# baekingeol/Probing-RAG

Measured on NVIDIA B200. Metric: bm25_top10_queries_per_sec, higher is better.
Workload: dtype f32

## Files before the change

include/probing_rag.h:

```cpp
#ifndef PROBING_RAG_H
#define PROBING_RAG_H

#include <stddef.h>
#include <stdint.h>

#ifdef __cplusplus
extern "C" {
#endif

#define PR_VERSION 201

#define PR_OK 0
#define PR_EINVAL (-1)
#define PR_ECUDA (-2)
#define PR_ERANGE (-3)
#define PR_EWORKSPACE (-4)
#define PR_EUNSUPPORTED (-5)

#define PR_MAX_K 128

typedef struct pr_index pr_index_t;
typedef void *pr_stream_t;

typedef struct pr_bm25_tuning {
// ... 38 lines not shown

int32_t pr_bm25_num_launches(const pr_index_t *index, int32_t n_queries, int32_t k, int64_t n_docs);
size_t pr_bm25_theta_offset(const pr_index_t *index, int32_t n_queries, int32_t k);
int pr_bm25_topk_range(pr_index_t *index, int32_t n_queries, const int64_t *q_indptr_dev,
                       const int32_t *q_terms_dev, int64_t n_q_terms, int32_t k, float *out_scores_dev,
                       int32_t *out_doc_ids_dev, void *workspace_dev, size_t workspace_bytes,
                       int32_t launch_begin, int32_t launch_end, pr_stream_t stream);

size_t pr_bm25_running_scores_offset(const pr_index_t *index, int32_t n_queries, int32_t k);
int pr_bm25_raise_union_bound(pr_index_t *index, int32_t n_queries, int32_t k, const float *gathered_scores_dev,
                              int32_t n_lists, void *workspace_dev, size_t workspace_bytes, pr_stream_t stream);

#define PR_MAX_PEERS 15
typedef struct pr_ipc_handle { unsigned char bytes[64]; } pr_ipc_handle_t;
int pr_peer_alloc(int device, size_t bytes, void **out_dev, pr_ipc_handle_t *out_handle);
int pr_peer_open(int device, const pr_ipc_handle_t *handle, void **out_dev);
int pr_peer_close(void *dev);
int pr_peer_free(void *dev);
int pr_index_set_peer_thetas(pr_index_t *index, float *local_dev, int64_t capacity, int32_t n_peers,
                             float *const *peer_bases_host, void *peer_table_dev);

int pr_bm25_status(const void *workspace_dev, pr_stream_t stream);

int pr_index_set_profiling(pr_index_t *index, int enable);
int pr_bm25_profile(pr_index_t *index, float *score_ms, int32_t *score_launches);

int64_t pr_bm25_last_launches(const pr_index_t *index);

int pr_topk_merge(int32_t n_queries, int32_t k, int32_t n_lists, const float *scores_dev,
                  const int32_t *ids_dev, float *out_scores_dev, int32_t *out_ids_dev,
                  pr_stream_t stream);

#define PR_PROBER_MAX 8

typedef struct pr_prober_set {
    int32_t n_probers;
    int32_t d_model;
    int32_t hidden;
    const float *w1_rowsum;
    const float *b1;
    const float *ln1_w, *ln1_b;
    const float *b2;
    const float *ln2_w, *ln2_b;
    const float *w3, *b3;
    const void *w1_hi, *w1_lo;
    const void *w2_hi, *w2_lo;
// ... 59 lines not shown
```

probing_rag_b200/_lib.py:

```python
from __future__ import annotations

import ctypes
import os

PKG_DIR = os.path.dirname(os.path.abspath(__file__))
LIB_PATH = os.environ.get("PR_LIB_PATH") or os.path.join(PKG_DIR, "libprobingrag.so")

PR_OK, PR_EINVAL, PR_ECUDA, PR_ERANGE, PR_EWORKSPACE, PR_EUNSUPPORTED = 0, -1, -2, -3, -4, -5
PR_MAX_K = 128
PR_PROBER_MAX = 8
PR_MAX_PEERS = 15
PR_FLAT_MAX_LISTS = 32
PR_METRIC_INNER_PRODUCT, PR_METRIC_L2 = 0, 1

c_i32, c_i64, c_f32, c_vp, c_sz = ctypes.c_int32, ctypes.c_int64, ctypes.c_float, ctypes.c_void_p, ctypes.c_size_t


class Tuning(ctypes.Structure):
    _fields_ = [("subs_per_item", c_i32), ("warps_per_cta", c_i32), ("docs_per_launch", c_i32),
                ("min_items", c_i32), ("items_per_warp", c_i32), ("tile_epochs", c_i32),
                ("batch_variant", c_i32)]


class AuxInfo(ctypes.Structure):
    _fields_ = [("table_rows", c_i32), ("hot_rows", c_i32), ("n_sub_tiles", c_i32),
                ("table_min_df", c_i64), ("hot_min_df", c_i64), ("hot_stream_bytes", c_i64),
                ("cold_stream_bytes", c_i64)]


class ProberSet(ctypes.Structure):
    _fields_ = [("n_probers", c_i32), ("d_model", c_i32), ("hidden", c_i32),
                ("w1_rowsum", c_vp), ("b1", c_vp),
                ("ln1_w", c_vp), ("ln1_b", c_vp), ("b2", c_vp),
                ("ln2_w", c_vp), ("ln2_b", c_vp), ("w3", c_vp), ("b3", c_vp),
                ("w1_hi", c_vp), ("w1_lo", c_vp), ("w2_hi", c_vp), ("w2_lo", c_vp)]


class FlatTuning(ctypes.Structure):
    _fields_ = [("first_chunk_rows", c_i64), ("growth", c_i32), ("cand_capacity", c_i32)]


class FlatStats(ctypes.Structure):
    _fields_ = [("launches", c_i64), ("chunks", c_i64), ("candidates", c_i64), ("max_candidates", c_i64),
                ("fallback_queries", c_i64)]


SIGNATURES = {
    "pr_version": (ctypes.c_int, []),
    "pr_last_error": (ctypes.c_char_p, []),
    "pr_index_create": (ctypes.c_int, [ctypes.POINTER(c_vp), ctypes.c_int, c_i64, c_i32, c_i32, c_i32, c_i64,
                                       c_vp, c_vp, c_vp]),
    "pr_index_destroy": (ctypes.c_int, [c_vp]),
    "pr_index_aux_bytes": (c_sz, [c_vp, c_sz]),
    "pr_index_build_aux": (ctypes.c_int, [c_vp, c_vp, c_sz, c_vp]),
    "pr_index_aux_info": (ctypes.c_int, [c_vp, ctypes.POINTER(AuxInfo)]),
    "pr_index_set_tuning": (ctypes.c_int, [c_vp, ctypes.POINTER(Tuning)]),
    "pr_index_get_tuning": (ctypes.c_int, [c_vp, ctypes.POINTER(Tuning)]),
    "pr_bm25_workspace_bytes": (c_sz, [c_vp, c_i32, c_i32]),
    "pr_bm25_topk": (ctypes.c_int, [c_vp, c_i32, c_vp, c_vp, c_i64, c_i32, c_vp, c_vp, c_vp, c_sz, c_vp]),
    "pr_bm25_num_launches": (c_i32, [c_vp, c_i32, c_i32, c_i64]),
    "pr_bm25_theta_offset": (c_sz, [c_vp, c_i32, c_i32]),
    "pr_bm25_running_scores_offset": (c_sz, [c_vp, c_i32, c_i32]),
    "pr_bm25_raise_union_bound": (ctypes.c_int, [c_vp, c_i32, c_i32, c_vp, c_i32, c_vp, c_sz, c_vp]),
    "pr_bm25_topk_range": (ctypes.c_int, [c_vp, c_i32, c_vp, c_vp, c_i64, c_i32, c_vp, c_vp, c_vp, c_sz, c_i32, c_i32,
                                          c_vp]),
    "pr_peer_alloc": (ctypes.c_int, [ctypes.c_int, c_sz, ctypes.POINTER(c_vp), ctypes.c_char_p]),
    "pr_peer_open": (ctypes.c_int, [ctypes.c_int, ctypes.c_char_p, ctypes.POINTER(c_vp)]),
    "pr_peer_close": (ctypes.c_int, [c_vp]),
    "pr_peer_free": (ctypes.c_int, [c_vp]),
    "pr_index_set_peer_thetas": (ctypes.c_int, [c_vp, c_vp, c_i64, c_i32, ctypes.POINTER(c_vp), c_vp]),
    "pr_bm25_status": (ctypes.c_int, [c_vp, c_vp]),
    "pr_bm25_last_launches": (c_i64, [c_vp]),
    "pr_index_set_profiling": (ctypes.c_int, [c_vp, ctypes.c_int]),
    "pr_bm25_profile": (ctypes.c_int, [c_vp, ctypes.POINTER(c_f32), ctypes.POINTER(c_i32)]),
    "pr_topk_merge": (ctypes.c_int, [c_i32, c_i32, c_i32, c_vp, c_vp, c_vp, c_vp, c_vp]),
    "pr_prober_workspace_bytes": (c_sz, [c_i32, c_i32, c_i32, c_i32]),
    "pr_pool_accumulate": (ctypes.c_int, [c_vp, c_i32, c_i32, c_i32, c_i32, c_vp, c_i32, c_i32, c_i32, c_i64, c_i64,
                                          c_vp, c_vp]),
    "pr_prober_forward": (ctypes.c_int, [ctypes.POINTER(ProberSet), c_i32, c_vp, c_i32, ctypes.c_double, c_i32, c_vp, c_vp,
                                         c_vp, c_vp, c_vp, c_vp, c_sz, c_vp]),
    "pr_flat_create": (ctypes.c_int, [ctypes.POINTER(c_vp), ctypes.c_int, c_vp, c_i64, c_i32]),
    "pr_flat_create_metric": (ctypes.c_int, [ctypes.POINTER(c_vp), ctypes.c_int, c_vp, c_i64, c_i32, ctypes.c_int]),
    "pr_flat_destroy": (ctypes.c_int, [c_vp]),
    "pr_flat_aux_bytes": (c_sz, [c_vp]),
    "pr_flat_build_aux": (ctypes.c_int, [c_vp, c_vp, c_sz, c_vp]),
    "pr_flat_set_tuning": (ctypes.c_int, [c_vp, ctypes.POINTER(FlatTuning)]),
    "pr_flat_get_tuning": (ctypes.c_int, [c_vp, ctypes.POINTER(FlatTuning)]),
    "pr_flat_workspace_bytes": (c_sz, [c_vp, c_i32, c_i32]),
    "pr_flat_search": (ctypes.c_int, [c_vp, c_i32, c_vp, c_i32, c_vp, c_vp, c_vp, c_sz, c_vp]),
    "pr_flat_last_stats": (ctypes.c_int, [c_vp, c_vp, c_i32, c_i32, ctypes.POINTER(FlatStats), c_vp]),
    "pr_flat_merge": (ctypes.c_int, [c_i32, c_i32, c_i32, c_vp, c_vp, ctypes.POINTER(c_i64), c_vp, c_vp, c_vp]),
    "pr_flat_merge_metric": (ctypes.c_int, [c_i32, c_i32, c_i32, c_vp, c_vp, ctypes.POINTER(c_i64), c_vp, c_vp, c_vp,
                                            ctypes.c_int]),
}
# ... 31 lines not shown
```

probing_rag_b200/csrc/bm25.cu:

```cuda
#include <string.h>

#include <vector>

#include "common.cuh"
#include "bm25_lean.cuh"
#include "bm25_kernels.h"

namespace {

__device__ __forceinline__ void fill_zero_tail(float *out_s, int32_t *out_d, int K, int nvalid, int doc_id_base, int n_docs)
{
    int cand = 0;
    for (int pos = nvalid; pos < K; ++pos) {
        while (cand < n_docs) {
            bool listed = false;
            for (int i = 0; i < nvalid; ++i)
                if (out_d[i] == cand + doc_id_base) listed = true;
            if (!listed) break;
            ++cand;
        }
        if (cand >= n_docs) break;
        out_s[pos] = 0.f;
        out_d[pos] = cand + doc_id_base;
        ++cand;
// ... 254 lines not shown
        const float *ps = gs + ((size_t)g * B + q) * K;
        bool done = false;
#pragma unroll
        for (int e = 0; e < E; ++e) {
            const int i0 = e * 32;
            if (done || i0 >= K) break;
            const float es = i0 + lane < K ? ps[i0 + lane] : -1.f;
            const int n = min(32, K - i0);
            for (int i = 0; i < n; ++i) {
                const float bs = __shfl_sync(PR_FULL_MASK, es, i);
                const int bd = g * K + i0 + i;
                if (bs < 0.f || !pr_beats(bs, bd, ks, kd)) {
                    done = true;
                    break;
                }
                L.insert(bs, bd, lane);
                L.kth(K, ks, kd);
            }
        }
    }
    if (ks > 0.f) prw::raise_theta(theta, nullptr, 0, q, ks, lane);
}

__global__ void bm25_init_kernel(float *run_s, int32_t *run_d, float *theta, int64_t n_run, int B, int32_t *counters,
                                 int n_counters, int32_t *status)
{
    const int64_t i = (int64_t)blockIdx.x * blockDim.x + threadIdx.x;
    if (i < n_run) {
        run_s[i] = PR_SENT_SCORE;
        run_d[i] = PR_SENT_DOC;
    }
    if (i < B && theta) theta[i] = PR_SENT_SCORE;
    if (i < n_counters) counters[i] = 0;
    if (i == 0) *status = 0;
}

__global__ void bm25_fill_kernel(float *p, int64_t n, float v)
{
    for (int64_t i = (int64_t)blockIdx.x * blockDim.x + threadIdx.x; i < n; i += (int64_t)gridDim.x * blockDim.x) p[i] = v;
}

__global__ void bm25_validate_kernel(const int64_t *indptr, const int32_t *doc_ids,
                                     const float *weights, int n_terms, int64_t nnz, int n_docs,
                                     int32_t *bad)
{
    const int64_t stride = (int64_t)gridDim.x * blockDim.x;
    const int64_t i0 = (int64_t)blockIdx.x * blockDim.x + threadIdx.x;
    for (int64_t t = i0; t < n_terms; t += stride) {
        const int64_t b = indptr[t], e = indptr[t + 1];
        if (b > e || b < 0 || e > nnz) atomicOr(bad, 1);
    }
    if (i0 == 0 && (indptr[0] != 0 || indptr[n_terms] != nnz)) atomicOr(bad, 1);
    uint32_t wmin = 0xffffffffu, wmax = 0u;
    for (int64_t p = i0; p < nnz; p += stride) {
        const int32_t d = doc_ids[p];
        const float w = weights[p];
        if (d < 0 || d >= n_docs) atomicOr(bad, 2);
// ... 23 lines not shown
}

}

constexpr int kNwChoices = 3;
constexpr int kEChoices = 3;

struct pr_index {
    int device;
    int64_t n_docs_global;
    int32_t doc_id_base, n_docs, n_terms;
    int64_t nnz;
    const int64_t *indptr;
    const int32_t *doc_ids;
    const float *weights;
    pr_bm25_tuning_t tuning;
    int num_sms;
    int64_t last_launches;
    int profiling;
    std::vector<cudaEvent_t> ev;
    int ev_used;
    const int32_t *heavy_row;
    const uint32_t *tp;
    int32_t n_rows, n_sub;
    int64_t heavy_min_df;
    const int32_t *hot_of_row;
    const uint32_t *hot_off;
    int32_t n_hot;
    int64_t hot_min_df, hot_stream_bytes;
    const unsigned char *cold_stream;
    uint32_t hot_base_g;
    int occ[kNwChoices][kEChoices][3];
    float max_weight;
    bool scale_ok;
    float *peer_local;
    float *const *peer_table;
    int32_t n_peers;
    int64_t peer_capacity;
    uint64_t peer_calls;
    int union_lists;
};

namespace {

struct Layout {
    int n_chunks, C, L;
// ... 157 lines not shown
    }
    pr_index *ix = new pr_index();
    memset(ix->occ, 0, sizeof(ix->occ));
    ix->peer_local = nullptr;
    ix->peer_table = nullptr;
    ix->n_peers = 0;
    ix->peer_capacity = 0;
    ix->peer_calls = 0;
    ix->union_lists = 1;
    ix->device = device;
    ix->n_docs_global = n_docs_global;
    ix->doc_id_base = doc_id_base;
    ix->n_docs = n_docs;
    ix->n_terms = n_terms;
    ix->nnz = nnz;
    ix->indptr = indptr_dev;
    ix->doc_ids = doc_ids_dev;
    ix->weights = weights_dev;
    ix->last_launches = 0;
    ix->profiling = 0;
    ix->ev_used = 0;
    ix->heavy_row = nullptr;
    ix->tp = nullptr;
    ix->n_rows = 0;
    ix->n_sub = (int32_t)(((int64_t)n_docs + prw::kSub - 1) >> prw::kSubShift);
    ix->heavy_min_df = 0;
    ix->hot_of_row = nullptr;
    ix->hot_off = nullptr;
    ix->n_hot = 0;
    ix->hot_min_df = 0;
    ix->hot_stream_bytes = 0;
    ix->cold_stream = nullptr;
    ix->hot_base_g = 0;
    {
        float wmin = 0.f, wmax = 0.f;
        if (nnz > 0) {
            memcpy(&wmin, &h_bad3[1], 4);
            memcpy(&wmax, &h_bad3[2], 4);
        }
        ix->max_weight = wmax;
        ix->scale_ok = nnz > 0 && wmin >= 9.313225746154785e-10f && wmax <= 256.f;
    }
    default_tuning(&ix->tuning);
    cudaDeviceProp prop;
    PR_CUDA_CHECK(cudaGetDeviceProperties(&prop, device));
    ix->num_sms = prop.multiProcessorCount;
    *out = ix;
    return PR_OK;
}

extern "C" int pr_index_destroy(pr_index_t *index)
{
    if (index)
        for (cudaEvent_t e : index->ev) cudaEventDestroy(e);
    delete index;
    return PR_OK;
}

extern "C" size_t pr_index_aux_bytes(const pr_index_t *index, size_t table_budget_bytes)
{
    if (!index) return 0;
    const size_t fixed = align_up((size_t)index->n_terms * 4, 256) + align_up(((size_t)index->n_terms / 1024 + 2) * 4, 256) + 256;
    return fixed + align_up((size_t)index->nnz * 8 + 256, 256) + align_up(table_budget_bytes, 256);
}

extern "C" int pr_index_build_aux(pr_index_t *index, void *aux_dev, size_t aux_bytes, pr_stream_t stream)
{
    if (!index || !aux_dev) {
        pr_set_error("pr_index_build_aux: null argument");
        return PR_EINVAL;
    }
    cudaStream_t st = (cudaStream_t)stream;
    const int nt = index->n_terms;
    const int n_blocks = (nt + 1023) / 1024;
    unsigned char *p = (unsigned char *)aux_dev;
    size_t o = 0;
    int32_t *heavy_row = (int32_t *)(p + o);  o = align_up(o + (size_t)nt * 4, 256);
    int32_t *block_cnt = (int32_t *)(p + o);  o = align_up(o + ((size_t)nt / 1024 + 2) * 4, 256);
    int32_t *count = (int32_t *)(p + o);      o += 256;
    unsigned char *cold = p + o;              o += align_up((size_t)index->nnz * 8 + 256, 256);
    if (o > aux_bytes) {
        pr_set_error("pr_index_build_aux: aux buffer of %zu bytes, need at least %zu (tables + 8 bytes per posting)", aux_bytes, o);
        return PR_EWORKSPACE;
    }
    const size_t budget = aux_bytes - o;
    size_t table_bytes = budget / 5;
    if (table_bytes < ((size_t)16 << 20)) table_bytes = budget < ((size_t)16 << 20) ? budget : ((size_t)16 << 20);
    const size_t per_row = ((size_t)index->n_sub + 1) * 4 + 4;
    int64_t min_df = prw::kLightDf;
    int32_t rows = 0;
    for (;;) {
        PR_CUDA_CHECK(cudaMemsetAsync(count, 0, 4, st));
        if (nt > 0) prw::count_heavy_kernel<<<296, 256, 0, st>>>(index->indptr, nt, min_df, count);
        PR_CUDA_CHECK(cudaGetLastError());
        PR_CUDA_CHECK(cudaMemcpyAsync(&rows, count, 4, cudaMemcpyDeviceToHost, st));
        PR_CUDA_CHECK(cudaStreamSynchronize(st));
        if ((size_t)rows * per_row + 1024 <= table_bytes || rows == 0) break;
        min_df *= 2;
    }
    int32_t *row_term = (int32_t *)(p + o);   o = align_up(o + (size_t)(rows > 0 ? rows : 1) * 4, 256);
    uint32_t *tp = (uint32_t *)(p + o);       o = align_up(o + (size_t)rows * ((size_t)index->n_sub + 1) * 4, 256);
    if (nt > 0) {
        prw::heavy_block_count_kernel<<<n_blocks, 1024, 0, st>>>(index->indptr, nt, min_df, block_cnt);
        prw::heavy_block_scan_kernel<<<1, 32, 0, st>>>(block_cnt, n_blocks);
        prw::heavy_assign_kernel<<<n_blocks, 1024, 0, st>>>(index->indptr, nt, min_df, block_cnt, heavy_row, row_term);
        if (rows > 0)
            prw::tp_fill_kernel<<<2368, 256, 0, st>>>(index->indptr, index->doc_ids, row_term, rows, index->n_sub, tp);
    }
    if (index->nnz > 0)
        prl::cold_fill_kernel<<<2368, 256, 0, st>>>(index->doc_ids, index->weights, index->nnz, (uint2 *)cold);
    PR_CUDA_CHECK(cudaGetLastError());
    PR_CUDA_CHECK(cudaStreamSynchronize(st));
    index->heavy_row = heavy_row;
    index->tp = tp;
    index->n_rows = rows;
    index->heavy_min_df = min_df;
    index->hot_of_row = nullptr;
    index->hot_off = nullptr;
    index->n_hot = 0;
    index->hot_min_df = 0;
    index->hot_stream_bytes = 0;
    index->cold_stream = cold;
    index->hot_base_g = 0;

    const int n_sub = index->n_sub;
    size_t oh = o;
    int32_t *hot_of_row = (int32_t *)(p + oh);  oh = align_up(oh + (size_t)(rows > 0 ? rows : 1) * 4, 256);
    int32_t *hot_rows = (int32_t *)(p + oh);    oh = align_up(oh + (size_t)(rows > 0 ? rows : 1) * 4, 256);
    int32_t *n_hot_dev = (int32_t *)(p + oh);
    uint32_t *total_dev = (uint32_t *)(p + oh + 64);
    oh += 256;
    if (rows == 0 || n_sub == 0 || oh + 4096 > aux_bytes) return PR_OK;
    int64_t hot_df = ((int64_t)prh::kHotMinSeg * index->n_docs + prw::kSub - 1) / prw::kSub;
    if (hot_df < min_df + 1) hot_df = min_df + 1;
    for (;; hot_df *= 2) {
        int32_t H = 0;
        prh::hot_assign_kernel<<<1, 32, 0, st>>>(index->indptr, row_term, rows, hot_df, hot_of_row, hot_rows, n_hot_dev);
// ... 224 lines not shown
    if (!index->heavy_row || !index->cold_stream) {
        pr_set_error("pr_bm25_topk: the index has no posting streams: call pr_index_build_aux first");
        return PR_EINVAL;
    }
    const Layout l = make_layout(index, n_queries, k);
    const int L = l.L > 0 ? l.L : 1;
    if (launch_begin < 0 || launch_end > L || launch_begin >= launch_end) {
        pr_set_error("pr_bm25_topk_range: launches [%d, %d) outside [0, %d)", launch_begin, launch_end, L);
        return PR_EINVAL;
    }
    if (workspace_bytes < l.total) {
        pr_set_error("pr_bm25_topk: workspace of %zu bytes, need %zu", workspace_bytes, l.total);
        return PR_EWORKSPACE;
    }
    if (launch_begin == 0) {
        index->last_launches = 0;
        index->ev_used = 0;
        index->union_lists = 1;
    }
    cudaStream_t st = (cudaStream_t)stream;
    unsigned char *ws = (unsigned char *)workspace_dev;
    int32_t *status = (int32_t *)(ws + l.off_status);
    if (n_queries == 0) {
        if (launch_begin == 0) PR_CUDA_CHECK(cudaMemsetAsync(status, 0, 4, st));
        return PR_OK;
    }
    const pr_bm25_tuning_t &t = index->tuning;
    const int E = e_of(k);
    int32_t *counters = (int32_t *)(ws + l.off_counters);
    float *theta = (float *)(ws + l.off_theta);
    float *theta_next = nullptr;
    float *const *peer_tab = nullptr;
    if (index->peer_local) {
        if (n_queries > index->peer_capacity) {
            pr_set_error("pr_bm25_topk: %d queries, the peer threshold arrays hold %lld", n_queries, (long long)index->peer_capacity);
            return PR_EINVAL;
        }
        if (launch_begin == 0) index->peer_calls++;
        const int parity = (int)(index->peer_calls & 1);
        theta = index->peer_local + (size_t)parity * index->peer_capacity;
        theta_next = index->peer_local + (size_t)(parity ^ 1) * index->peer_capacity;
        peer_tab = index->peer_table + parity * PR_MAX_PEERS;
    }
    const int n_peers = index->peer_local ? index->n_peers : 0;
    float *run_s = (float *)(ws + l.off_run_s);
    int32_t *run_d = (int32_t *)(ws + l.off_run_d);
    float *part_s = (float *)(ws + l.off_part_s);
// ... 47 lines not shown
    w.tp = index->tp;
    w.hot_of_row = index->hot_of_row;
    w.hot_off = index->hot_off;
    w.stream_base = index->cold_stream;
    w.hot_base_g = index->hot_base_g;
    w.cursors = (uint32_t *)(ws + l.off_cursors);
    w.q_indptr = q_indptr_dev;
    w.q_terms = q_terms_dev;
    w.theta = theta;
    w.peer_theta = peer_tab;
    w.n_peers = n_peers;
    w.part_s = part_s;
    w.part_d = part_d;
    w.status = status;
    w.n_q_terms = n_q_terms;
    w.n_docs = index->n_docs;
    w.n_terms = index->n_terms;
    w.doc_id_base = index->doc_id_base;
    w.n_queries = n_queries;
    w.K = k;
    w.n_sub = index->n_sub;
    w.subs_per_item = l.G;
    w.max_weight = index->max_weight;

    for (int li = launch_begin; li < launch_end; ++li) {
        const int chunk0 = l.launch_chunk0[li], Cl = l.launch_chunks[li];
        const int64_t items = (int64_t)n_queries * Cl;
        const int64_t seen = (int64_t)chunk0 * l.G * prw::kSub * index->union_lists;
        const int late = l.L > 1 && (li > first_full || (index->union_lists > 1 && seen >= (int64_t)81920 * k)) ? 1 : 0;
        const score_fn_t fn = fns[late];
        int64_t grid = (int64_t)occs[late] * index->num_sms;
        const int64_t need = (items + nw - 1) / nw;
        if (grid > need) grid = need;
        if (index->profiling) {
            while ((int)index->ev.size() < index->ev_used + 2) {
                cudaEvent_t ev;
                PR_CUDA_CHECK(cudaEventCreate(&ev));
                index->ev.push_back(ev);
            }
            PR_CUDA_CHECK(cudaEventRecord(index->ev[index->ev_used], st));
        }
        w.chunk0 = chunk0;
        w.n_chunks_launch = Cl;
        w.counter = counters + li;
        fn<<<(unsigned)grid, threads, smem, st>>>(w);
        PR_CUDA_CHECK(cudaGetLastError());
// ... 19 lines not shown
                              workspace_dev, workspace_bytes, 0, L > 0 ? L : 1, stream);
}

extern "C" int pr_bm25_status(const void *workspace_dev, pr_stream_t stream)
{
    if (!workspace_dev) {
        pr_set_error("pr_bm25_status: null workspace");
        return PR_EINVAL;
    }
    int32_t h = 0;
    PR_CUDA_CHECK(cudaMemcpyAsync(&h, workspace_dev, 4, cudaMemcpyDeviceToHost, (cudaStream_t)stream));
    PR_CUDA_CHECK(cudaStreamSynchronize((cudaStream_t)stream));
    if (h & 2) {
        pr_set_error("query CSR inconsistent: q_indptr must start at 0, be non-decreasing and end within q_terms");
        return PR_EINVAL;
    }
    if (h & 1) {
        pr_set_error("query term id outside [0, n_terms)");
        return PR_ERANGE;
    }
    return PR_OK;
}

extern "C" int pr_topk_merge(int32_t n_queries, int32_t k, int32_t n_lists, const float *scores_dev,
                             const int32_t *ids_dev, float *out_scores_dev, int32_t *out_ids_dev,
                             pr_stream_t stream)
{
    if (n_queries < 0 || n_lists < 1 || !scores_dev || !ids_dev || !out_scores_dev || !out_ids_dev) {
        pr_set_error("pr_topk_merge: bad argument");
        return PR_EINVAL;
    }
    if (k < 1 || k > PR_MAX_K) {
        pr_set_error("pr_topk_merge: k must be in [1, %d] (got %d)", PR_MAX_K, k);
        return PR_EINVAL;
    }
    if (n_queries == 0) return PR_OK;
    return launch_merge(e_of(k), (cudaStream_t)stream, scores_dev, ids_dev, n_lists, k, (int64_t)n_queries * k, nullptr,
                        nullptr, nullptr, nullptr, 0, n_queries, k, 1, out_scores_dev, out_ids_dev, 0, -1);
}
```

probing_rag_b200/csrc/bm25_lean.cuh:

```cuda
#pragma once

#include "bm25_hot.cuh"

#ifndef PR_LEAN_FOLD
#define PR_LEAN_FOLD 6
#endif
#ifndef PR_LEAN_PIPE
#define PR_LEAN_PIPE 2
#endif
#ifndef PR_LEAN_CTAS
#define PR_LEAN_CTAS 3
#endif
#ifndef PR_LEAN_SIGN_EPOCH
#define PR_LEAN_SIGN_EPOCH 1
#endif
#ifndef PR_LEAN_L2HINT
#define PR_LEAN_L2HINT 2
#endif
#include <type_traits>

namespace prl {

using prw::kSub;
using prw::kSubShift;
using prw::ScoreArgs;

constexpr int kScanLimit = 4;
constexpr int kTileWords = kSub + 32 + 4;

__device__ __forceinline__ float lds_f32(uint32_t a)
{
    float v;
    asm volatile("ld.shared.f32 %0, [%1];" : "=f"(v) : "r"(a) : "memory");
    return v;
}
__device__ __forceinline__ void sts_f32(uint32_t a, float v) { asm volatile("st.shared.f32 [%0], %1;" ::"r"(a), "f"(v) : "memory"); }
__device__ __forceinline__ uint2 lds_u2(uint32_t a)
{
    uint2 v;
    asm volatile("ld.shared.v2.u32 {%0, %1}, [%2];" : "=r"(v.x), "=r"(v.y) : "r"(a) : "memory");
    return v;
}
__device__ __forceinline__ uint4 ldg_stream_u4(const void *p)
{
    uint4 r;
    asm volatile("ld.global.nc.L1::no_allocate.v4.u32 {%0, %1, %2, %3}, [%4];" : "=r"(r.x), "=r"(r.y), "=r"(r.z), "=r"(r.w) : "l"(p));
    return r;
}
__device__ __forceinline__ float4 ldg_stream_f4(const void *p)
{
    float4 r;
// ... 43 lines not shown
                 : "=f"(r.x), "=f"(r.y), "=f"(r.z), "=f"(r.w) : "l"(p), "l"(pol));
    return r;
}
__device__ __forceinline__ uint32_t ldg_hint_u1(const void *p, uint64_t pol)
{
    uint32_t r;
    asm volatile("ld.global.nc.L1::no_allocate.L2::cache_hint.u32 %0, [%1], %2;" : "=r"(r) : "l"(p), "l"(pol));
    return r;
}
__device__ __forceinline__ void sts_u2(uint32_t a, uint32_t x, uint32_t y)
{
    asm volatile("st.shared.v2.u32 [%0], {%1, %2};" ::"r"(a), "r"(x), "r"(y) : "memory");
}
__device__ __forceinline__ int uni(int v) { return __reduce_max_sync(PR_FULL_MASK, v); }

static __global__ void __launch_bounds__(256) cold_fill_kernel(const int32_t *__restrict__ doc_ids, const float *__restrict__ weights,
                                                        int64_t nnz, uint2 *__restrict__ cold)
{
    const int64_t stride = (int64_t)gridDim.x * blockDim.x;
    for (int64_t p = (int64_t)blockIdx.x * blockDim.x + threadIdx.x; p < nnz; p += stride)
        cold[p] = make_uint2((uint32_t)(doc_ids[p] & (kSub - 1)) * 4u, __float_as_uint(weights[p]));
}

constexpr float kEpochScale = 1.2089258196146292e+24f;
constexpr float kEpochUnscale = 8.271806125530277e-25f;
constexpr float kEpochCut = 8.881784197001252e-16f;
constexpr float kEpochMaxSum = 16777216.f;

template <int NW, int E, int VAR>
__global__ void __launch_bounds__(NW * 32, (NW <= 4 ? 2 * PR_LEAN_CTAS : NW <= 8 ? PR_LEAN_CTAS : NW <= 12 ? 2 : 1))
    bm25_lean_kernel(const ScoreArgs a)
{
    constexpr bool REFRESH = VAR == 1;
    constexpr int kEpochs = VAR == 2 ? 4 : 2;
    constexpr bool kFold = (PR_LEAN_FOLD >> VAR) & 1;
    extern __shared__ __align__(16) unsigned char smem_raw[];
    int lane = threadIdx.x & 31;
    const int warp = threadIdx.x >> 5;
    asm volatile("" : "+r"(lane));
    unsigned char *smem_al = smem_raw + ((1024u - ((uint32_t)__cvta_generic_to_shared(smem_raw) & 1023u)) & 1023u);
    uint2 *desc = reinterpret_cast<uint2 *>(smem_al) + warp * kRing;
    float *tile = reinterpret_cast<float *>(smem_al + (size_t)NW * kRing * 8) + warp * kTileWords;
    float4 *tile4 = reinterpret_cast<float4 *>(tile);
    const float4 zero4 = make_float4(0.f, 0.f, 0.f, 0.f);
    uint32_t tile_sa = (uint32_t)__cvta_generic_to_shared(tile);
    uint32_t desc_sa = (uint32_t)__cvta_generic_to_shared(desc);
    asm volatile("" : "+r"(tile_sa), "+r"(desc_sa));
    const uint32_t dummy_off = (uint32_t)kSub * 4u;
    const unsigned char *const sbase = a.stream_base;
    const unsigned char *wide_base = sbase + lane * 16, *narrow_base = sbase + lane * 8;
    asm volatile("" : "+l"(wide_base), "+l"(narrow_base));
#if PR_LEAN_L2HINT
    uint64_t l2_keep;
    asm volatile("createpolicy.fractional.L2::evict_last.b64 %0, 1.0;" : "=l"(l2_keep));
#endif
    const uint32_t hot_base_g = a.hot_base_g;

#pragma unroll
    for (int v = lane & 31; v < kTileWords / 4; v += 32) tile4[v] = zero4;
    __syncwarp();

    const int K = a.K, C = a.n_chunks_launch, G = a.subs_per_item;
    const int64_t n_items = (int64_t)a.n_queries * C;
    const size_t tab_stride = (size_t)a.n_sub + 1;
    WarpTopK<E> item;

    auto slot = [&](int pos) -> uint32_t { return desc_sa | (((uint32_t)pos << 3) & (uint32_t)(kRing * 8 - 8)); };

    while (true) {
        int item_i = 0;
        if (lane == 0) item_i = atomicAdd(a.counter, 1);
        item_i = __shfl_sync(PR_FULL_MASK, item_i, 0);
        if ((int64_t)item_i >= n_items) break;
        const int c = item_i / a.n_queries, q = item_i - c * a.n_queries;
        const int64_t qb = a.q_indptr[q];
        int nq = (int)min(a.q_indptr[q + 1] - qb, (int64_t)0x7fffffff);
        if (qb < 0 || nq < 0 || qb + nq > a.n_q_terms || (q == 0 && qb != 0)) {
            if (lane == 0) atomicOr(a.status, 2);
            nq = 0;
        }
        float *const theta_q = a.theta + q;
        float theta_pub = ld_theta(theta_q);
        const uint32_t stash_sa = tile_sa + (uint32_t)(kSub + 32) * 4u;
        if (!REFRESH) sts_f32(stash_sa, theta_pub);
        item.reset();
        float thr = fmaxf(theta_pub, PR_DENORM_MIN);
        float iks = PR_SENT_SCORE;
        int ikd = PR_SENT_DOC;
        const int sub0 = (a.chunk0 + c) * G;
        const int sub1 = min(sub0 + G, a.n_sub);
        const bool single = nq <= 32;
        float mx = 0.f;

        int t_class = -1;
        int64_t t_b0 = 0;
        int32_t t_row = 0;
        uint32_t tb_cur = 0, tb_next = 0;
        int32_t t_pos = 0, t_le = 0, t_nd = 0x7fffffff;

        int32_t t_df = 0;
        auto load_info = [&](int p0, int np, int dlo, int dhi) {
            t_class = -1;
            t_b0 = 0;
            t_row = 0;
            t_pos = 0;
            t_le = 0;
// ... 20 lines not shown
                }
            }
            t_df = df;
            const bool rare = t_class == 0 && df > 0;
            unsigned sm = __ballot_sync(PR_FULL_MASK, rare);
            while (sm) {
                const int j = __ffs(sm) - 1;
                sm &= sm - 1;
                const int64_t b0 = __shfl_sync(PR_FULL_MASK, t_b0, j);
                const int64_t e0 = b0 + __shfl_sync(PR_FULL_MASK, df, j);
                const int64_t lo = pr_lower_bound_warp(a.doc_ids, b0, e0, dlo, lane);
                int64_t lim = lo + (dhi - dlo);
                if (lim > e0) lim = e0;
                const int64_t hi = pr_lower_bound_warp(a.doc_ids, lo, lim, dhi, lane);
                if (lane == j) {
                    t_pos = (int32_t)(lo - b0);
                    t_le = (int32_t)(hi - b0);
                }
            }
            if (rare && t_pos < t_le) t_nd = __ldg(a.doc_ids + t_b0 + t_pos);
        };

        if (single && nq > 0) load_info(0, nq, sub0 << kSubShift, min(sub1 << kSubShift, a.n_docs));
        uint32_t *const cur_w = a.cursors ? a.cursors + (size_t)(blockIdx.x * NW + warp) * (kCursorCap * kCursorWords) : nullptr;
        uint4 *const info_w = reinterpret_cast<uint4 *>(cur_w + kCursorCap);
        const bool multi = !single && cur_w != nullptr && nq <= kCursorCap;
        if (multi) {
            const int item_lo = sub0 << kSubShift, item_hi = min(sub1 << kSubShift, a.n_docs);
            for (int p0 = 0; p0 < nq; p0 += 32) {
                load_info(p0, min(32, nq - p0), item_lo, item_hi);
                if (p0 + lane < nq) {
                    cur_w[p0 + lane] = (uint32_t)t_pos;
                    info_w[p0 + lane] = make_uint4((uint32_t)t_b0, (uint32_t)((uint64_t)t_b0 >> 32),
                                                   ((uint32_t)(t_class + 1) << 28) | ((uint32_t)t_row & 0x0fffffffu), (uint32_t)t_df);
                }
            }
        }
        auto load_cached = [&](int p0, int np) {
            t_class = -1;
            t_b0 = 0;
            t_row = 0;
            t_pos = 0;
            t_le = 0;
            t_nd = 0x7fffffff;
            if (lane < np) {
                const uint4 w = info_w[p0 + lane];
// ... 353 lines not shown
            } else {
                const uint32_t o = b.d.x;
                const float x = lds_f32(tile_sa + o);
                const float w = __uint_as_float(b.d.y);
                const float v = acc(x, w, ep_c);
                sts_f32(tile_sa + o, v);
                mx = NEG ? fminf(mx, v) : fmaxf(mx, v);
            }
        };
        auto end_subtile = [&](const uint32_t meta) {
            const int g_end = (int)((meta & ~(uint32_t)kFlagWide) >> kSubIdxShift);
            const int base_doc = (g_end << kSubShift) + a.doc_id_base;
            auto consider = [&](float bs, int off) {
                const int bd = base_doc + off;
                if (bs >= thr && pr_beats(bs, bd, iks, ikd)) {
                    item.insert(bs, bd, lane);
                    item.kth(K, iks, ikd);
                    thr = fmaxf(thr, iks);
                }
            };
            const int ep = (hd >> kEpShift) & 3;
            const float unscale = (ep == 1 || ep == 2 ? -1.f : 1.f) * (ep >= 2 ? kEpochUnscale : 1.f);
            const float peak = mx * unscale;
            bool scan = __any_sync(PR_FULL_MASK, peak >= thr);
            if (scan) {
                const float t = REFRESH ? ld_theta(theta_q) : lds_f32(tile_sa + dummy_off);
                if (t > thr) {
                    thr = t;
                    scan = __any_sync(PR_FULL_MASK, peak >= thr);
                }
                if (REFRESH) theta_pub = fmaxf(theta_pub, t);
            }
            if (!scan) {
                if (ep == ep_last || !PR_LEAN_SIGN_EPOCH) {
#pragma unroll
                    for (int vv = lane & 31; vv < kSub / 4; vv += 32) tile4[vv] = zero4;
                    hd &= ~kEpMask;
                } else {
                    hd += 1 << kEpShift;
                }
            } else {
                const float cut = ep >= 2 ? kEpochCut : -1.f;
#pragma unroll 4
                for (int vv = lane & 31; vv < kSub / 4; vv += 32) {
                    const float4 xb = tile4[vv];
                    tile4[vv] = zero4;
                    float xs[4] = {xb.x * unscale, xb.y * unscale, xb.z * unscale, xb.w * unscale};
#pragma unroll
                    for (int cc = 0; cc < 4; ++cc) xs[cc] = xs[cc] >= cut ? xs[cc] : 0.f;
                    const float m4 = fmaxf(fmaxf(xs[0], xs[1]), fmaxf(xs[2], xs[3]));
                    if (__any_sync(PR_FULL_MASK, m4 >= thr)) {
#pragma unroll
                        for (int cc = 0; cc < 4; ++cc) {
                            unsigned mm = __ballot_sync(PR_FULL_MASK, xs[cc] >= thr);
                            while (mm) {
                                const int l = __ffs(mm) - 1;
                                mm &= mm - 1;
                                consider(__shfl_sync(PR_FULL_MASK, xs[cc], l), 4 * (vv - (lane & 31) + l) + cc);
                            }
                        }
                    }
                }
                hd &= ~kEpMask;
            }
            mx = 0.f;
            if (REFRESH && iks > theta_pub) {
                raise_theta(a.theta, a.peer_theta, a.n_peers, q, iks, lane);
                theta_pub = iks;
            }
            __syncwarp();
        };
        auto round = [&](auto ep_c) -> uint32_t {
            uint32_t meta_last = 0u;
#pragma unroll
            for (int d = 0; d < kPipe; ++d) {
                const uint2 ds = lds_u2(slot(hd + d + kPipe));
                if (d == kPipe - 1) meta_last = buf[d].meta;
                rmw(buf[d], ep_c);
                issue(ds, buf[d]);
            }
            hd += kPipe;
            return meta_last;
        };
// ... 59 lines not shown
```

probing_rag_b200/csrc/bm25_tables.cuh:

```cuda
#pragma once

#include "common.cuh"

#ifndef PR_SUB_SHIFT
#define PR_SUB_SHIFT 11
#endif

namespace prw {

__device__ __forceinline__ float ld_theta(const float *p)
{
    float v;
    asm volatile("ld.relaxed.sys.global.f32 %0, [%1];" : "=f"(v) : "l"(p) : "memory");
    return v;
}
__device__ __forceinline__ void raise_theta(float *local, float *const *peer_theta, int n_peers, int q, float v, int lane)
{
    if (lane == 0) {
        atomicMax(reinterpret_cast<int *>(local + q), __float_as_int(v));
    } else if (lane <= n_peers) {
        int *dst = reinterpret_cast<int *>(peer_theta[lane - 1] + q);
        asm volatile("red.relaxed.sys.global.max.s32 [%0], %1;" ::"l"(dst), "r"(__float_as_int(v)) : "memory");
    }
}
// ... 6 lines not shown
    const int64_t *__restrict__ indptr;
    const int32_t *__restrict__ doc_ids;
    const float *__restrict__ weights;
    const int32_t *__restrict__ heavy_row;
    const uint32_t *__restrict__ tp;
    const int32_t *__restrict__ hot_of_row;
    const uint32_t *__restrict__ hot_off;
    const unsigned char *__restrict__ stream_base;
    uint32_t hot_base_g;
    uint32_t *cursors;
    const int64_t *__restrict__ q_indptr;
    const int32_t *__restrict__ q_terms;
    float *theta;
    float *const *peer_theta;
    int32_t n_peers;
    float *part_s;
    int32_t *part_d;
    int32_t *counter;
    int32_t *status;
    int64_t n_q_terms;
    int32_t n_docs, n_terms, doc_id_base, n_queries, K;
    int32_t n_sub, subs_per_item, chunk0, n_chunks_launch;
    float max_weight;
};

static __global__ void count_heavy_kernel(const int64_t *indptr, int n_terms, int64_t min_df, int32_t *count)
{
    int local = 0;
    for (int64_t t = (int64_t)blockIdx.x * blockDim.x + threadIdx.x; t < n_terms; t += (int64_t)gridDim.x * blockDim.x)
        local += (indptr[t + 1] - indptr[t]) > min_df;
    for (int o = 16; o; o >>= 1) local += __shfl_down_sync(PR_FULL_MASK, local, o);
    if ((threadIdx.x & 31) == 0 && local) atomicAdd(count, local);
}

static __global__ void heavy_block_count_kernel(const int64_t *indptr, int n_terms, int64_t min_df, int32_t *block_cnt)
{
    __shared__ int s;
    if (threadIdx.x == 0) s = 0;
    __syncthreads();
    const int64_t t = (int64_t)blockIdx.x * blockDim.x + threadIdx.x;
    const int flag = t < n_terms && (indptr[t + 1] - indptr[t]) > min_df;
    const unsigned m = __ballot_sync(PR_FULL_MASK, flag);
    if ((threadIdx.x & 31) == 0 && m) atomicAdd(&s, __popc(m));
    __syncthreads();
    if (threadIdx.x == 0) block_cnt[blockIdx.x] = s;
}
// ... 53 lines not shown
```

probing_rag_b200/index.py:

```python
from __future__ import annotations

import ctypes
import json
import math
import os

import numpy as np
import torch

from . import _lib

K1 = 1.5
B = 0.75


def idf_lucene_table(df: np.ndarray, n_docs: int) -> np.ndarray:
    df = np.asarray(df, dtype=np.int64)
    uniq, inv = np.unique(df, return_inverse=True)
    table = np.array([math.log(1 + (n_docs - int(v) + 0.5) / (int(v) + 0.5)) if v > 0 else 0.0
                      for v in uniq], dtype=np.float64)
    return table[inv].reshape(df.shape).astype(np.float32)


def count_postings(tokens: torch.Tensor, doc_lens: torch.Tensor, vocab: int):
# ... 247 lines not shown
                rounds = n_launch - 1 if exchange_rounds is None else max(int(exchange_rounds), n_launch - 1)
                done = 0
                for li in range(n_launch):
                    _lib.check(L.pr_bm25_topk_range(*args, li, li + 1, stream))
                    if done < rounds:
                        exchange(theta)
                        done += 1
                for _ in range(rounds - done):
                    exchange(theta)
            if check_status and nq:
                _lib.check(L.pr_bm25_status(ws.data_ptr(), stream))
        return out

    def num_launches(self, n_queries: int, k: int, n_docs: int | None = None) -> int:
        n = int(_lib.lib().pr_bm25_num_launches(self._handle, n_queries, k, -1 if n_docs is None else int(n_docs)))
        if n < 0:
            raise ValueError(f"k must be in [1, {_lib.PR_MAX_K}] (got {k})")
        return n

    def check_status(self, n_queries: int, k: int) -> None:
        _lib.check(_lib.lib().pr_bm25_status(self._workspace(n_queries, k).data_ptr(),
                                              torch.cuda.current_stream(self.device).cuda_stream))

    def topk_host(self, q_indptr: np.ndarray, q_terms: np.ndarray, k: int, exchange=None):
        d_qi, d_qt, n_terms = self._stage_queries(q_indptr, q_terms)
        s, d = self.topk(d_qi, d_qt, k, check_status=False, exchange=exchange)
        h_s, h_d = self._unstage_lists(s, d)
        _lib.check(_lib.lib().pr_bm25_status(self._workspace(len(q_indptr) - 1, k).data_ptr(),
                                              torch.cuda.current_stream(self.device).cuda_stream))
        return h_s.numpy().copy(), h_d.numpy().copy(), (len(q_indptr)) * 8 + n_terms * 4, (len(q_indptr) - 1) * k * 8

    def _stage_queries(self, q_indptr: np.ndarray, q_terms: np.ndarray):
        q_indptr = np.asarray(q_indptr)
        q_terms = np.asarray(q_terms)
        if q_indptr.ndim != 1 or len(q_indptr) < 1 or q_terms.ndim != 1:
            raise ValueError("q_indptr must be a 1-D array of n_queries+1 offsets and q_terms 1-D")
        n_i, n_t = len(q_indptr), len(q_terms)
        st = self._pinned
        if st.get("qi") is None or st["qi"].numel() < n_i:
            st["qi"] = torch.empty(max(n_i, 1024), dtype=torch.int64).pin_memory()
        if st.get("qt") is None or st["qt"].numel() < max(n_t, 1):
            st["qt"] = torch.empty(max(n_t, 4096), dtype=torch.int32).pin_memory()
        st["qi"].numpy()[:n_i] = q_indptr
        st["qt"].numpy()[:n_t] = q_terms
        d_qi = st["qi"][:n_i].to(self.device, non_blocking=True)
        d_qt = st["qt"][:n_t].to(self.device, non_blocking=True)
# ... 31 lines not shown
```

Before: 157,000.

## Skip low-impact query terms via per-term max-weight bound and rescore candidates

Adds a per-term max-weight table built at aux time. In the lean scoring kernel, a query's lowest-weight terms whose summed max weights stay below half of theta are dropped from accumulation. Accumulated peaks are then checked against an upper bound (partial score plus skipped mass). Surviving candidates are rescored exactly by binary-searching each query term's postings, and skip counters are exposed via a stats API. This trades fewer posting reads for extra binary-search rescoring, a larger aux buffer and more shared scratch words.

```diff
diff --git a/include/probing_rag.h b/include/probing_rag.h
--- a/include/probing_rag.h
+++ b/include/probing_rag.h
@@ -84,6 +84,13 @@
 
 int pr_bm25_status(const void *workspace_dev, pr_stream_t stream);
 
+typedef struct pr_bm25_stats {
+    int64_t skipped_terms;
+    int64_t skipped_postings;
+    int64_t rescored;
+} pr_bm25_stats_t;
+int pr_bm25_last_stats(const void *workspace_dev, pr_bm25_stats_t *out, pr_stream_t stream);
+
 int pr_index_set_profiling(pr_index_t *index, int enable);
 int pr_bm25_profile(pr_index_t *index, float *score_ms, int32_t *score_launches);
 
diff --git a/probing_rag_b200/_lib.py b/probing_rag_b200/_lib.py
--- a/probing_rag_b200/_lib.py
+++ b/probing_rag_b200/_lib.py
@@ -36,6 +36,10 @@
                 ("w1_hi", c_vp), ("w1_lo", c_vp), ("w2_hi", c_vp), ("w2_lo", c_vp)]
 
 
+class BM25Stats(ctypes.Structure):
+    _fields_ = [("skipped_terms", c_i64), ("skipped_postings", c_i64), ("rescored", c_i64)]
+
+
 class FlatTuning(ctypes.Structure):
     _fields_ = [("first_chunk_rows", c_i64), ("growth", c_i32), ("cand_capacity", c_i32)]
 
@@ -70,6 +74,7 @@
     "pr_peer_free": (ctypes.c_int, [c_vp]),
     "pr_index_set_peer_thetas": (ctypes.c_int, [c_vp, c_vp, c_i64, c_i32, ctypes.POINTER(c_vp), c_vp]),
     "pr_bm25_status": (ctypes.c_int, [c_vp, c_vp]),
+    "pr_bm25_last_stats": (ctypes.c_int, [c_vp, ctypes.POINTER(BM25Stats), c_vp]),
     "pr_bm25_last_launches": (c_i64, [c_vp]),
     "pr_index_set_profiling": (ctypes.c_int, [c_vp, ctypes.c_int]),
     "pr_bm25_profile": (ctypes.c_int, [c_vp, ctypes.POINTER(c_f32), ctypes.POINTER(c_i32)]),
diff --git a/probing_rag_b200/csrc/bm25.cu b/probing_rag_b200/csrc/bm25.cu
--- a/probing_rag_b200/csrc/bm25.cu
+++ b/probing_rag_b200/csrc/bm25.cu
@@ -300,6 +300,8 @@
     if (ks > 0.f) prw::raise_theta(theta, nullptr, 0, q, ks, lane);
 }
 
+__host__ __device__ inline unsigned long long *skip_stats_of(int32_t *status) { return reinterpret_cast<unsigned long long *>(status + 2); }
+
 __global__ void bm25_init_kernel(float *run_s, int32_t *run_d, float *theta, int64_t n_run, int B, int32_t *counters,
                                  int n_counters, int32_t *status)
 {
@@ -311,6 +313,7 @@
     if (i < B && theta) theta[i] = PR_SENT_SCORE;
     if (i < n_counters) counters[i] = 0;
     if (i == 0) *status = 0;
+    if (i < 3) skip_stats_of(status)[i] = 0;
 }
 
 __global__ void bm25_fill_kernel(float *p, int64_t n, float v)
@@ -380,6 +383,7 @@
     int ev_used;
     const int32_t *heavy_row;
     const uint32_t *tp;
+    const float *term_maxw;
     int32_t n_rows, n_sub;
     int64_t heavy_min_df;
     const int32_t *hot_of_row;
@@ -583,6 +587,7 @@
     ix->ev_used = 0;
     ix->heavy_row = nullptr;
     ix->tp = nullptr;
+    ix->term_maxw = nullptr;
     ix->n_rows = 0;
     ix->n_sub = (int32_t)(((int64_t)n_docs + prw::kSub - 1) >> prw::kSubShift);
     ix->heavy_min_df = 0;
@@ -621,7 +626,7 @@
 extern "C" size_t pr_index_aux_bytes(const pr_index_t *index, size_t table_budget_bytes)
 {
     if (!index) return 0;
-    const size_t fixed = align_up((size_t)index->n_terms * 4, 256) + align_up(((size_t)index->n_terms / 1024 + 2) * 4, 256) + 256;
+    const size_t fixed = 2 * align_up((size_t)index->n_terms * 4, 256) + align_up(((size_t)index->n_terms / 1024 + 2) * 4, 256) + 256;
     return fixed + align_up((size_t)index->nnz * 8 + 256, 256) + align_up(table_budget_bytes, 256);
 }
 
@@ -637,6 +642,7 @@
     unsigned char *p = (unsigned char *)aux_dev;
     size_t o = 0;
     int32_t *heavy_row = (int32_t *)(p + o);  o = align_up(o + (size_t)nt * 4, 256);
+    float *term_maxw = (float *)(p + o);      o = align_up(o + (size_t)nt * 4, 256);
     int32_t *block_cnt = (int32_t *)(p + o);  o = align_up(o + ((size_t)nt / 1024 + 2) * 4, 256);
     int32_t *count = (int32_t *)(p + o);      o += 256;
     unsigned char *cold = p + o;              o += align_up((size_t)index->nnz * 8 + 256, 256);
@@ -670,10 +676,12 @@
     }
     if (index->nnz > 0)
         prl::cold_fill_kernel<<<2368, 256, 0, st>>>(index->doc_ids, index->weights, index->nnz, (uint2 *)cold);
+    if (nt > 0) prl::term_maxw_kernel<<<2368, 256, 0, st>>>(index->indptr, index->weights, nt, term_maxw);
     PR_CUDA_CHECK(cudaGetLastError());
     PR_CUDA_CHECK(cudaStreamSynchronize(st));
     index->heavy_row = heavy_row;
     index->tp = tp;
+    index->term_maxw = term_maxw;
     index->n_rows = rows;
     index->heavy_min_df = min_df;
     index->hot_of_row = nullptr;
@@ -944,7 +952,7 @@
     unsigned char *ws = (unsigned char *)workspace_dev;
     int32_t *status = (int32_t *)(ws + l.off_status);
     if (n_queries == 0) {
-        if (launch_begin == 0) PR_CUDA_CHECK(cudaMemsetAsync(status, 0, 4, st));
+        if (launch_begin == 0) PR_CUDA_CHECK(cudaMemsetAsync(status, 0, 32, st));
         return PR_OK;
     }
     const pr_bm25_tuning_t &t = index->tuning;
@@ -1038,6 +1046,8 @@
     w.n_sub = index->n_sub;
     w.subs_per_item = l.G;
     w.max_weight = index->max_weight;
+    w.term_maxw = index->term_maxw;
+    w.skip_stats = skip_stats_of(status);
 
     for (int li = launch_begin; li < launch_end; ++li) {
         const int chunk0 = l.launch_chunk0[li], Cl = l.launch_chunks[li];
@@ -1103,6 +1113,21 @@
     return PR_OK;
 }
 
+extern "C" int pr_bm25_last_stats(const void *workspace_dev, pr_bm25_stats_t *out, pr_stream_t stream)
+{
+    if (!workspace_dev || !out) {
+        pr_set_error("pr_bm25_last_stats: null argument");
+        return PR_EINVAL;
+    }
+    unsigned long long h[3];
+    PR_CUDA_CHECK(cudaMemcpyAsync(h, skip_stats_of((int32_t *)workspace_dev), sizeof(h), cudaMemcpyDeviceToHost, (cudaStream_t)stream));
+    PR_CUDA_CHECK(cudaStreamSynchronize((cudaStream_t)stream));
+    out->skipped_terms = (int64_t)h[0];
+    out->skipped_postings = (int64_t)h[1];
+    out->rescored = (int64_t)h[2];
+    return PR_OK;
+}
+
 extern "C" int pr_topk_merge(int32_t n_queries, int32_t k, int32_t n_lists, const float *scores_dev,
                              const int32_t *ids_dev, float *out_scores_dev, int32_t *out_ids_dev,
                              pr_stream_t stream)
diff --git a/probing_rag_b200/csrc/bm25_lean.cuh b/probing_rag_b200/csrc/bm25_lean.cuh
--- a/probing_rag_b200/csrc/bm25_lean.cuh
+++ b/probing_rag_b200/csrc/bm25_lean.cuh
@@ -26,7 +26,19 @@
 using prw::ScoreArgs;
 
 constexpr int kScanLimit = 4;
-constexpr int kTileWords = kSub + 32 + 4;
+constexpr int kTileWords = kSub + 32 + 8;
+enum : int { kStashTheta = kSub + 32, kStashSkipM, kStashSkipOcc, kStashCands, kStashPostings  };
+static_assert(kStashPostings % 2 == 0 && kTileWords % 4 == 0, "scratch alignment");
+
+constexpr float kSkipGamma1 = 1.000003814697265625f;
+#ifndef PR_SKIP
+#define PR_SKIP 1
+#endif
+#ifndef PR_SKIP_FRAC
+#define PR_SKIP_FRAC 0.5f
+#endif
+constexpr float kSkipFrac = PR_SKIP_FRAC;
+static_assert(kSkipFrac > 0.f && kSkipFrac <= 1.f, "M must stay below theta");
 
 __device__ __forceinline__ float lds_f32(uint32_t a)
 {
@@ -116,6 +128,20 @@
         cold[p] = make_uint2((uint32_t)(doc_ids[p] & (kSub - 1)) * 4u, __float_as_uint(weights[p]));
 }
 
+static __global__ void __launch_bounds__(256) term_maxw_kernel(const int64_t *__restrict__ indptr, const float *__restrict__ weights,
+                                                        int n_terms, float *__restrict__ term_maxw)
+{
+    const int lane = threadIdx.x & 31;
+    const int64_t n_warps = (int64_t)gridDim.x * (blockDim.x >> 5);
+    for (int64_t t = ((int64_t)blockIdx.x * blockDim.x + threadIdx.x) >> 5; t < n_terms; t += n_warps) {
+        const int64_t e = indptr[t + 1];
+        uint32_t m = 0;
+        for (int64_t p = indptr[t] + lane; p < e; p += 32) m = max(m, __float_as_uint(weights[p]));
+        m = __reduce_max_sync(PR_FULL_MASK, m);
+        if (lane == 0) term_maxw[t] = __uint_as_float(m);
+    }
+}
+
 constexpr float kEpochScale = 1.2089258196146292e+24f;
 constexpr float kEpochUnscale = 8.271806125530277e-25f;
 constexpr float kEpochCut = 8.881784197001252e-16f;
@@ -126,6 +152,7 @@
     bm25_lean_kernel(const ScoreArgs a)
 {
     constexpr bool REFRESH = VAR == 1;
+    constexpr bool kSkip = !REFRESH && PR_SKIP;
     constexpr int kEpochs = VAR == 2 ? 4 : 2;
     constexpr bool kFold = (PR_LEAN_FOLD >> VAR) & 1;
     extern __shared__ __align__(16) unsigned char smem_raw[];
@@ -165,7 +192,17 @@
         int item_i = 0;
         if (lane == 0) item_i = atomicAdd(a.counter, 1);
         item_i = __shfl_sync(PR_FULL_MASK, item_i, 0);
-        if ((int64_t)item_i >= n_items) break;
+        if ((int64_t)item_i >= n_items) {
+            if (kSkip && lane == 0) {
+                const uint32_t occ = __float_as_uint(lds_f32(tile_sa + kStashSkipOcc * 4u));
+                const uint32_t cands = __float_as_uint(lds_f32(tile_sa + kStashCands * 4u));
+                const uint2 post = lds_u2(tile_sa + kStashPostings * 4u);
+                if (occ) atomicAdd(a.skip_stats + 0, (unsigned long long)occ);
+                if (post.x | post.y) atomicAdd(a.skip_stats + 1, ((unsigned long long)post.y << 32) | post.x);
+                if (cands) atomicAdd(a.skip_stats + 2, (unsigned long long)cands);
+            }
+            break;
+        }
         const int c = item_i / a.n_queries, q = item_i - c * a.n_queries;
         const int64_t qb = a.q_indptr[q];
         int nq = (int)min(a.q_indptr[q + 1] - qb, (int64_t)0x7fffffff);
@@ -175,7 +212,7 @@
         }
         float *const theta_q = a.theta + q;
         float theta_pub = ld_theta(theta_q);
-        const uint32_t stash_sa = tile_sa + (uint32_t)(kSub + 32) * 4u;
+        const uint32_t stash_sa = tile_sa + (uint32_t)kStashTheta * 4u;
         if (!REFRESH) sts_f32(stash_sa, theta_pub);
         item.reset();
         float thr = fmaxf(theta_pub, PR_DENORM_MIN);
@@ -242,6 +279,38 @@
         };
 
         if (single && nq > 0) load_info(0, nq, sub0 << kSubShift, min(sub1 << kSubShift, a.n_docs));
+        if (kSkip) {
+            float skip_m = 0.f;
+            if (single && theta_pub > 0.f) {
+                const float w = t_class >= 1 ? __ldg(a.term_maxw + a.q_terms[qb + lane]) : __int_as_float(0x7f800000);
+                float pm = 0.f;
+#pragma unroll 1
+                for (int j = 0; j < 32; ++j) {
+                    const float wj = __shfl_sync(PR_FULL_MASK, w, j);
+                    if (wj < w || (wj == w && j <= lane)) pm = __fadd_ru(pm, wj);
+                }
+                const bool skip = t_class >= 1 && __fmul_ru(pm, kSkipGamma1) < kSkipFrac * theta_pub;
+                skip_m = __uint_as_float(__reduce_max_sync(PR_FULL_MASK, skip ? __float_as_uint(pm) : 0u));
+                const unsigned sk = __ballot_sync(PR_FULL_MASK, skip);
+                if (sk) {
+                    uint32_t n_post = 0;
+                    if (skip) {
+                        const uint32_t *tab = a.tp + (size_t)__ldg(a.heavy_row + a.q_terms[qb + lane]) * tab_stride;
+                        n_post = __ldg(tab + sub1) - __ldg(tab + sub0);
+                        t_class = -1;
+                    }
+                    n_post = __reduce_add_sync(PR_FULL_MASK, n_post);
+                    if (lane == 0) {
+                        const uint32_t occ_sa = tile_sa + kStashSkipOcc * 4u, post_sa = tile_sa + kStashPostings * 4u;
+                        sts_f32(occ_sa, __uint_as_float(__float_as_uint(lds_f32(occ_sa)) + __popc(sk)));
+                        const uint2 pv = lds_u2(post_sa);
+                        const unsigned long long tot = (((unsigned long long)pv.y << 32) | pv.x) + n_post;
+                        sts_u2(post_sa, (uint32_t)tot, (uint32_t)(tot >> 32));
+                    }
+                }
+            }
+            sts_f32(tile_sa + kStashSkipM * 4u, skip_m);
+        }
         uint32_t *const cur_w = a.cursors ? a.cursors + (size_t)(blockIdx.x * NW + warp) * (kCursorCap * kCursorWords) : nullptr;
         uint4 *const info_w = reinterpret_cast<uint4 *>(cur_w + kCursorCap);
         const bool multi = !single && cur_w != nullptr && nq <= kCursorCap;
@@ -641,12 +710,14 @@
             const int ep = (hd >> kEpShift) & 3;
             const float unscale = (ep == 1 || ep == 2 ? -1.f : 1.f) * (ep >= 2 ? kEpochUnscale : 1.f);
             const float peak = mx * unscale;
-            bool scan = __any_sync(PR_FULL_MASK, peak >= thr);
+            const float skip_m = kSkip ? lds_f32(tile_sa + kStashSkipM * 4u) : 0.f;
+            auto bound = [&](float p) -> float { return skip_m > 0.f ? __fmul_ru(__fadd_ru(p, skip_m), kSkipGamma1) : p; };
+            bool scan = __any_sync(PR_FULL_MASK, bound(peak) >= thr);
             if (scan) {
                 const float t = REFRESH ? ld_theta(theta_q) : lds_f32(tile_sa + dummy_off);
                 if (t > thr) {
                     thr = t;
-                    scan = __any_sync(PR_FULL_MASK, peak >= thr);
+                    scan = __any_sync(PR_FULL_MASK, bound(peak) >= thr);
                 }
                 if (REFRESH) theta_pub = fmaxf(theta_pub, t);
             }
@@ -660,6 +731,7 @@
                 }
             } else {
                 const float cut = ep >= 2 ? kEpochCut : -1.f;
+                unsigned long long cand = 0ull;
 #pragma unroll 4
                 for (int vv = lane & 31; vv < kSub / 4; vv += 32) {
                     const float4 xb = tile4[vv];
@@ -668,7 +740,12 @@
 #pragma unroll
                     for (int cc = 0; cc < 4; ++cc) xs[cc] = xs[cc] >= cut ? xs[cc] : 0.f;
                     const float m4 = fmaxf(fmaxf(xs[0], xs[1]), fmaxf(xs[2], xs[3]));
-                    if (__any_sync(PR_FULL_MASK, m4 >= thr)) {
+                    if (kSkip && skip_m > 0.f) {
+                        uint32_t c4 = 0;
+#pragma unroll
+                        for (int cc = 0; cc < 4; ++cc) c4 |= (bound(xs[cc]) >= thr ? 1u : 0u) << cc;
+                        cand |= (unsigned long long)c4 << ((vv >> 5) * 4);
+                    } else if (__any_sync(PR_FULL_MASK, m4 >= thr)) {
 #pragma unroll
                         for (int cc = 0; cc < 4; ++cc) {
                             unsigned mm = __ballot_sync(PR_FULL_MASK, xs[cc] >= thr);
@@ -678,6 +755,50 @@
                                 consider(__shfl_sync(PR_FULL_MASK, xs[cc], l), 4 * (vv - (lane & 31) + l) + cc);
                             }
                         }
+                    }
+                }
+                if (kSkip) {
+                    int n_cands = 0;
+#pragma unroll 1
+                    while (__any_sync(PR_FULL_MASK, cand != 0ull)) {
+                        float sc = 0.f;
+                        int off = 0;
+                        n_cands += __popc(__ballot_sync(PR_FULL_MASK, cand != 0ull));
+                        if (cand) {
+                            const int b = __ffsll((long long)cand) - 1;
+                            cand &= cand - 1;
+                            off = 4 * (lane + 32 * (b >> 2)) + (b & 3);
+                            const int d = (g_end << kSubShift) + off;
+#pragma unroll 1
+                            for (int p = 0; p < nq; ++p) {
+                                const int32_t t = __ldg(a.q_terms + qb + p);
+                                if (t < 0 || t >= a.n_terms) continue;
+                                int64_t lo = __ldg(a.indptr + t), hi = __ldg(a.indptr + t + 1);
+                                const int row = __ldg(a.heavy_row + t);
+                                if (row >= 0) {
+                                    const uint32_t *tab = a.tp + (size_t)row * tab_stride + g_end;
+                                    hi = lo + __ldg(tab + 1);
+                                    lo += __ldg(tab);
+                                }
+                                const int64_t e = hi;
+                                while (lo < hi) {
+                                    const int64_t mid = (lo + hi) >> 1;
+                                    if (__ldg(a.doc_ids + mid) < d) lo = mid + 1;
+                                    else hi = mid;
+                                }
+                                if (lo < e && __ldg(a.doc_ids + lo) == d) sc = sc + __ldg(a.weights + lo);
+                            }
+                        }
+                        unsigned mm = __ballot_sync(PR_FULL_MASK, sc >= thr);
+                        while (mm) {
+                            const int l = __ffs(mm) - 1;
+                            mm &= mm - 1;
+                            consider(__shfl_sync(PR_FULL_MASK, sc, l), __shfl_sync(PR_FULL_MASK, off, l));
+                        }
+                    }
+                    if (n_cands && lane == 0) {
+                        const uint32_t cs = tile_sa + kStashCands * 4u;
+                        sts_f32(cs, __uint_as_float(__float_as_uint(lds_f32(cs)) + (uint32_t)n_cands));
                     }
                 }
                 hd &= ~kEpMask;
diff --git a/probing_rag_b200/csrc/bm25_tables.cuh b/probing_rag_b200/csrc/bm25_tables.cuh
--- a/probing_rag_b200/csrc/bm25_tables.cuh
+++ b/probing_rag_b200/csrc/bm25_tables.cuh
@@ -52,6 +52,8 @@
     int32_t n_docs, n_terms, doc_id_base, n_queries, K;
     int32_t n_sub, subs_per_item, chunk0, n_chunks_launch;
     float max_weight;
+    const float *__restrict__ term_maxw;
+    unsigned long long *skip_stats;
 };
 
 static __global__ void count_heavy_kernel(const int64_t *indptr, int n_terms, int64_t min_df, int32_t *count)
diff --git a/probing_rag_b200/index.py b/probing_rag_b200/index.py
--- a/probing_rag_b200/index.py
+++ b/probing_rag_b200/index.py
@@ -293,6 +293,12 @@
         _lib.check(_lib.lib().pr_bm25_status(self._workspace(n_queries, k).data_ptr(),
                                               torch.cuda.current_stream(self.device).cuda_stream))
 
+    def last_stats(self, n_queries: int, k: int) -> dict:
+        s = _lib.BM25Stats()
+        _lib.check(_lib.lib().pr_bm25_last_stats(self._workspace(n_queries, k).data_ptr(), ctypes.byref(s),
+                                                  torch.cuda.current_stream(self.device).cuda_stream))
+        return {f: int(getattr(s, f)) for f, _ in _lib.BM25Stats._fields_}
+
     def topk_host(self, q_indptr: np.ndarray, q_terms: np.ndarray, k: int, exchange=None):
         d_qi, d_qt, n_terms = self._stage_queries(q_indptr, q_terms)
         s, d = self.topk(d_qi, d_qt, k, check_status=False, exchange=exchange)
```

New measurement: 68230 (median of 6 runs). 56.5% lower.
